# gundoganalperen/DIRAL

Measured on AMD Instinct MI355X. Metric: agent-steps/sec (envs x vehicles), 64-UE/32-res batched env, higher is better.
Workload: dtype f64

## Files before the change

diral_amd/_lib.py:

```python
from __future__ import annotations

import ctypes
import os

from .config import DiralCfg

HERE = os.path.dirname(os.path.abspath(__file__))
LIB_PATH = os.environ.get("DIRAL_LIB") or os.path.join(HERE, "libdiral_env.so")

SYMBOLS = [
    "diral_cfg_defaults", "diral_env_state_space", "diral_env_validate", "diral_env_strerror",
    "diral_env_abi_version", "diral_env_create", "diral_env_destroy", "diral_env_hbm_bytes",
    "diral_env_reset", "diral_env_step", "diral_env_observe", "diral_env_update_velocity",
    "diral_env_sample", "diral_env_info_age", "diral_env_export_state", "diral_env_import_state",
    "diral_env_metrics", "diral_env_check", "diral_env_last_hip_error", "diral_sps_step", "diral_sps_init",
    "diral_env_set_trace", "diral_env_set_option", "diral_env_last_kernel",
    "diral_sps_window_from_chobs", "diral_sps_step_chobs", "diral_driver_shape",
    "diral_env_export_entries", "diral_env_import_entries",
    "diral_env_set_clock", "diral_clock_add", "diral_sps_step_chobs_clocked", "diral_env_step_policy",
    "diral_env_set_capture_rotation", "diral_env_align_phase",
    "diral_env_export_prev_obs", "diral_env_import_prev_obs", "diral_env_prefill", "diral_env_prefill_mode",
    "diral_env_rollout",
]

_lib = None


class DiralLibraryError(RuntimeError):
    pass


def load() -> ctypes.CDLL:
    global _lib
    if _lib is not None:
        return _lib
# ... 32 lines not shown
        "diral_env_last_hip_error": (ctypes.c_char_p, [P]),
        "diral_sps_step": (I, [I, I, P, P, P, D, D, D, P, P, P, U64, P, P]),
        "diral_sps_init": (I, [I, I, P, P, U64, P]),
        "diral_env_set_trace": (I, [P, P, I, I, P]),
        "diral_env_set_option": (I, [P, I, I64]),
        "diral_env_last_kernel": (I, [P]),
        "diral_sps_window_from_chobs": (I, [I, I, P, I, P, P, P]),
        "diral_sps_step_chobs": (I, [I, I, P, I, P, P, P, D, D, D, P, P, P, U64, P, P]),
        "diral_driver_shape": (I, [I, I, I, P, I, P, P, P, P, P, I, I, D, P, P, P, P, P, P]),
        "diral_env_set_clock": (I, [P, P]),
        "diral_clock_add": (I, [P, I64, P]),
        "diral_sps_step_chobs_clocked": (I, [I, I, P, I, P, P, P, D, D, D, U64, P, P, P]),
        "diral_env_step_policy": (I, [P, I, P, I64, P, P, P, P, I, P, P]),
        "diral_env_set_capture_rotation": (I, [P, I, P]),
        "diral_env_align_phase": (I, [P, I, P]),
        "diral_env_export_prev_obs": (I, [P, P, P]),
        "diral_env_import_prev_obs": (I, [P, P, P]),
        "diral_env_prefill": (I, [P, P, I, U64, P, I, P, P, P, D, D, P]),
        "diral_env_prefill_mode": (I, [P, I, P, I, U64, P, I, P, P, P, D, D, P]),
        "diral_env_rollout": (I, [P, I, P, I, I64, P, I, P, P, I, P, P]),
    }
    for name in SYMBOLS:
        try:
            fn = getattr(lib, name)
        except AttributeError as exc:
            raise DiralLibraryError("libdiral_env.so lacks symbol %s" % name) from exc
        fn.restype, fn.argtypes = sig[name]
    from .config import ABI_VERSION
    got = int(lib.diral_env_abi_version())
    if got != ABI_VERSION:
# ... 9 lines not shown
```

diral_amd/csrc/diral_env.hip:

```cpp
#include <hip/hip_runtime.h>

#include <cmath>
#include <cstdio>
#include <cstdlib>
#include <cstring>
#include <string>
#include <vector>

#include "aux_kernels.hpp"
#include "common.hpp"
#include "launch.hpp"
#include "observe_kernel.hpp"
#include "piggyback_kernel.hpp"
#include "posdist_kernel.hpp"
#include "step_params.hpp"

using namespace diral;

struct DevBuf {
  void* p;
  size_t bytes;
  size_t reset_bytes;
  int fill;
};
constexpr int kNoFill = -1;
constexpr bool kOnReset = true;

struct Hooks {
  int table_form = 0;
  bool no_fast64 = false;
  bool no_wide = false;
  bool slow_first = true;
  bool wide_slow_first = false;
  int f32_margin = -1;
};

struct DiralEnv {
  DiralCfg cfg;
  Hooks hooks;
  std::vector<DevBuf> bufs;
  int B = 0, N = 0, A = 0, K = 0, S = 0, NV = 0, NR = 0, vpl = 1;
  int device = 0;
  StepParams base;
  RichParams rich;
  uint32_t lds_bytes = 0;
  int64_t env_offset = 0;
  int kernel_path = DIRAL_PATH_AUTO;
  int last_kernel = -1;
  double* pos_x = nullptr;
  double* pos_y = nullptr;
  double* vel = nullptr;
  uint32_t* tkey = nullptr;
  double* tx = nullptr;
  double* ring = nullptr;
  bool plane_valid = true, ring_valid = false;
  uint32_t* tcode = nullptr;
  uint32_t* tage = nullptr;
  uint32_t* tseq = nullptr;
  uint32_t* told = nullptr;
  uint32_t* slow = nullptr;
  uint64_t slow_launches = 0;
  bool capture_rotates = false;
  int32_t* la = nullptr;
  int32_t* pf = nullptr;
  double* metrics = nullptr;
  uint32_t* err = nullptr;
  double* edges = nullptr;
  double* edges1 = nullptr;
  double* inv_tab = nullptr;
  double* trace = nullptr;
  int trace_len = 0, trace_per_env = 0;
  bool flat_y = true;
  uint32_t* yflag = nullptr;
  int off_chobs_pb = -1;
  double* prev_obs = nullptr;
  double* obs_new = nullptr;
  int32_t* txid = nullptr;
// ... 72 lines not shown
  const int vpl = vpl_for(c->num_users);
  return lds_layout(64 * vpl, c->num_channels, c->num_bins > 0 ? c->num_bins : 1, vpl, 4 * vpl).total > 160u * 1024u;
}
bool runs_large(const DiralEnv* e) { return e->large || e->kernel_path == DIRAL_PATH_LARGE; }

bool fits_fast64(const DiralEnv* e) { return !e->large && e->vpl == 1 && e->NV == 64 && e->A <= kFastMaxA; }
bool fits_wide(const DiralEnv* e) { return !e->large && e->vpl > 1 && e->A <= kWideMaxA; }

Hooks read_hooks() {
  Hooks h;
  if (const char* f = std::getenv("DIRAL_TABLE_FORM")) h.table_form = std::strcmp(f, "packed") == 0 ? 1 : (std::strcmp(f, "plane") == 0 ? -1 : 0);
  h.no_fast64 = std::getenv("DIRAL_NO_FAST64") != nullptr;
  h.no_wide = std::getenv("DIRAL_NO_WIDE") != nullptr;
  if (const char* off = std::getenv("DIRAL_NO_SLOW_FIRST")) h.slow_first = off[0] != '1';
  if (const char* ws = std::getenv("DIRAL_WIDE_SLOW_FIRST")) h.wide_slow_first = ws[0] == '1';
  if (const char* fm = std::getenv("DIRAL_F32_MARGIN")) h.f32_margin = std::max(0, std::atoi(fm));
  return h;
}

constexpr double kPackedMinNeighbours = 20.0;
constexpr double kPackedMinNeighbours2 = 15.0;
bool use_packed_table(const DiralEnv* e) {
  if (e->vpl == 1) return true;
  if (e->hooks.table_form != 0) return e->hooks.table_form > 0;
  const double neigh = e->N * 2.0 * e->cfg.communication_range / e->cfg.highway_length;
  return neigh >= (e->vpl == 2 ? kPackedMinNeighbours2 : kPackedMinNeighbours);
}

int device_of_ptr(const void* p) {
  hipPointerAttribute_t a;
// ... 238 lines not shown
  f.chobs_mode = (p.chobs_out ? 1 : 0) | ((p.mode == DIRAL_STEP_MY_STEP && p.state_type == 2) ? 2 : 0);
  f.L = p.L; f.Rc = p.Rc; f.Rb = p.Rb; f.inv_w = p.hist_inv_width; f.t = p.t; f.t_dev = p.t_dev;
  f.actions = p.actions; f.pos_x = p.pos_x; f.pos_y = p.pos_y; f.vel = p.vel; f.tkey = p.tkey; f.tx = p.tx;
  f.metrics = p.metrics; f.err = p.err; f.edges = p.edges; f.inv_tab = e->inv_tab;
  f.ring = d.use_ring ? e->ring : nullptr;
  f.tcode = e->tcode; f.tage = e->tage; f.tseq = e->tseq; f.told = e->told;
  f.la = d.la;
  f.trace_len = p.trace_len; f.trace_per_env = p.trace_per_env;
  f.state_out = p.state_out; f.rew_out = p.rew_out;
  f.done_out = p.done_out; f.dbg = p.dbg;
  f.B = p.B;
  f.f32_m16 = d.use_fast64 ? f32_margin16(p.L, p.Rb, p.K, e->hooks.f32_margin) : 0;
  f.f32_xmax = (float)p.L;
  f.slow_cnt_r = nullptr; f.slow_list_r = nullptr; f.slow_flag_r = nullptr;
  f.slow_cnt_w = nullptr; f.slow_list_w = nullptr; f.slow_flag_w = nullptr; f.slow_cnt_z = nullptr;
  return f;
}

void rotate_slow_sets(DiralEnv* e, FastParams& f, hipStream_t s) {
  const size_t w = slow_set_words(e);
  uint32_t* const set_r = e->slow + (e->slow_launches % 3) * w;
  uint32_t* const set_w = e->slow + ((e->slow_launches + 1) % 3) * w;
  uint32_t* const set_z = e->slow + ((e->slow_launches + 2) % 3) * w;
  f.slow_cnt_r = set_r; f.slow_list_r = set_r + 16; f.slow_flag_r = set_r + 16 + fast_slow_max(e->B);
  if (e->capture_rotates || !stream_is_capturing(s)) {
    f.slow_cnt_w = set_w; f.slow_list_w = set_w + 16; f.slow_flag_w = set_w + 16 + fast_slow_max(e->B);
    f.slow_cnt_z = set_z;
    ++e->slow_launches;
  }
}

hipError_t launch_step_any(DiralEnv* e, const StepParams& p, const StepPlan& d, hipStream_t s, const PolParams* pol = nullptr) {
  const hipError_t st = d.use_ring ? ensure_ring(e, s) : ensure_plane(e, s);
  if (st != hipSuccess) return st;
  if (d.use_ring) e->plane_valid = false;
  else if (p.mode != kModeObserve) e->ring_valid = false;
  e->last_kernel = d.last_kernel;
  if (d.launch == StepLaunch::Large) return launch_large(p, e->lg, s);
  if (d.launch == StepLaunch::General) return launch_general(e->vpl, d.general_fast, p, e->lds_bytes, s);
  FastParams f = fast_params(e, p, d);
  if (d.slow_sets) rotate_slow_sets(e, f, s);
  RichParams r = rich_for(e, p);
  r.chobs_out = p.chobs_out;
  r.pf = ((p.flags & DIRAL_F_PROPORTIONAL_FAIR) && p.mode == DIRAL_STEP_MY_STEP) ? p.pf : nullptr;
  r.pf_threshold = p.pf_threshold; r.pf_penalty = p.pf_penalty;
  const int grid = p.B + (d.slow_sets ? fast_slow_max(p.B) : 0);
  switch (d.launch) {
    case StepLaunch::WideSlots: return launch_wide_slots(f, r, *pol, d.k, e->vpl, p.B, s);
    case StepLaunch::Wide: return e->vpl == 2 ? launch_wide2(f, r, d.k, grid, s) : launch_wide4(f, r, d.k, grid, s);
    case StepLaunch::Fast64Slots: return launch_fast64_slots(f, r, *pol, d.k.ch, d.k.out64, p.B, s);
    case StepLaunch::Fast64Policy: return launch_fast64_policy(f, r, *pol, d.k.out64, grid, s);
    default: return launch_fast64(f, r, d.k, grid, s);
  }
}

hipError_t launch_posdist_if_needed(DiralEnv* e, const StepParams& p, hipStream_t s) {
  const bool full = (p.flags & DIRAL_F_ADD_POSDIST) != 0;
  const bool type1 = (p.flags & DIRAL_F_ADD_POSDIST_PIGGY) && p.posdist_type == 1;
  if (!p.state_out || !(full || type1)) return hipSuccess;
  PosdistParams q;
  q.N = p.N; q.A = p.A; q.K = p.K; q.S = p.S; q.NV = p.NV; q.NR = p.NR; q.flags = p.flags;
// ... 196 lines not shown
  CREATE_TRY(own(e, e->pos_y, bn * 8));
  CREATE_TRY(own(e, e->vel, bn * 8));
  const size_t tab_slack = 512 + 64 * 256;
  CREATE_TRY(own(e, e->tkey, tab * 4, tab_slack * 4, kOnReset));
  CREATE_TRY(own(e, e->tx, tab * 8, tab_slack * 8, kOnReset));
  if (fits_fast64(e) || fits_wide(e)) {
    CREATE_TRY(own(e, e->ring, (size_t)e->B * e->NR * 8 * 8, 0, kOnReset));
    if (use_packed_table(e)) {
      const size_t nq = (size_t)e->B * (e->NR / 4);
      CREATE_TRY(own(e, e->tcode, nq * e->NV * 4, 512 * 4, kOnReset));
      CREATE_TRY(own(e, e->tage, nq * e->NV * 4, 512 * 4, kOnReset));
      CREATE_TRY(own(e, e->tseq, (size_t)e->B * e->NR * 4, 64 * 4, kOnReset));
      CREATE_TRY(own(e, e->told, nq * 4, 16 * 4, kOnReset));
    }
    CREATE_TRY(own(e, e->slow, 3 * slow_set_words(e) * 4, 0, kOnReset));
    e->ring_valid = true;
  }
  CREATE_TRY(own(e, e->metrics, (size_t)e->B * DIRAL_M_COLUMNS * 8, 0, kOnReset));
  CREATE_TRY(own(e, e->err, 4));
  CREATE_TRY(own(e, e->yflag, 4, 0, false, kNoFill));
  CREATE_TRY(own(e, e->edges, (size_t)(e->K + 1) * 8, 0, false, kNoFill));
  CREATE_TRY(own(e, e->edges1, (size_t)(e->K + 1) * 8, 0, false, kNoFill));
  CREATE_TRY(own(e, e->inv_tab, 256 * 8, 0, false, kNoFill));
  if (has(cfg, DIRAL_F_TRACK_ARRIVAL)) CREATE_TRY(own(e, e->la, bn * e->N * 4, 0, kOnReset, 0xFF));
  if (has(cfg, DIRAL_F_PROPORTIONAL_FAIR)) CREATE_TRY(own(e, e->pf, bn * 4, 0, kOnReset));
  if (has(cfg, DIRAL_F_PIGGYBACKING)) {
    if (piggy_search_lds_bytes(e->N) > 48u * 1024u)
      CREATE_TRY(hipFuncSetAttribute(reinterpret_cast<const void*>(piggy_search_kernel), hipFuncAttributeMaxDynamicSharedMemorySize,
                                     (int)piggy_search_lds_bytes(e->N)));
    CREATE_TRY(own(e, e->prev_obs, bn * e->A * 8, 0, kOnReset));
// ... 66 lines not shown
  r.off_act = off.act; r.off_chobs = has(cfg, DIRAL_F_PIGGYBACKING) ? -1 : off.chobs; r.off_hist = off.hist; r.off_rew = off.rew; r.off_idx = off.idx;
  r.off_skip = 0; r.len_skip = 0;
  r.off_pos = off.pos; r.off_vel = off.vel; r.off_fp = off.fp;
  r.H = cfg->highway_height; r.vel = e->vel; r.pos_y = e->pos_y;
  if (e->hooks.no_fast64 && e->vpl == 1) e->kernel_path = DIRAL_PATH_GENERAL;
  if (e->hooks.no_wide && e->vpl > 1 && !e->large) e->kernel_path = DIRAL_PATH_GENERAL;
  *out = e;
  return DIRAL_OK;
}

int diral_env_destroy(DiralEnv* e) {
  if (!e) return DIRAL_OK;
  DeviceGuard guard(e->device);
  for (const DevBuf& b : e->bufs) (void)hipFree(b.p);
  if (e->trace) (void)hipFree(e->trace);
  if (e->dbg) (void)hipFree(e->dbg);
  delete e;
  return DIRAL_OK;
}

int64_t diral_env_hbm_bytes(const DiralEnv* e) {
  int64_t sum = 0;
  if (e) for (const DevBuf& b : e->bufs) sum += (int64_t)b.bytes;
  return sum;
}

int diral_env_set_option(DiralEnv* e, int option, int64_t value) {
  if (!e) return DIRAL_ERR_BAD_ARG;
  switch (option) {
    case DIRAL_OPT_ENV_OFFSET:
// ... 16 lines not shown
}

int diral_env_last_kernel(const DiralEnv* e) { return e ? e->last_kernel : DIRAL_ERR_BAD_ARG; }

const char* diral_env_last_hip_error(const DiralEnv* e) { return e ? e->last_hip_error.c_str() : ""; }

int diral_env_reset(DiralEnv* e, const double* x0, const double* y0, const double* v0, uint64_t seed,
                    void* stream) {
  if (!e) return DIRAL_ERR_BAD_ARG;
  DEVICE_ENTER(e->device);
  hipStream_t s = (hipStream_t)stream;
  const size_t bn = (size_t)e->B * e->N;
  for (const DevBuf& b : e->bufs)
    if (b.reset_bytes) HIP_TRY(e, hipMemsetAsync(b.p, b.fill, b.reset_bytes, s));
  e->slow_launches = 0;
  e->plane_valid = true; e->ring_valid = e->ring != nullptr;
  HIP_TRY(e, launch_1d<reset_kernel>(bn, s, (int)bn, e->cfg.highway_length, has(&e->cfg, DIRAL_F_MOBILITY_VARY) ? 1 : 0, seed,
                                     (uint64_t)e->env_offset * (uint64_t)e->N, x0, y0, v0, e->pos_x, e->pos_y, e->vel));
  if (y0) { if (refresh_flat_y(e, s) != DIRAL_OK) return DIRAL_ERR_HIP; }
  else e->flat_y = true;
  return DIRAL_OK;
}

int diral_env_step(DiralEnv* e, int mode, const int32_t* actions, int64_t t, void* state_out, void* rew_out,
                   uint8_t* done_out, void* chobs_out, int out_dtype, double episode, double epsilon,
                   void* stream) {
  if (!e || !actions) return DIRAL_ERR_BAD_ARG;
  if (mode != DIRAL_STEP_MY_STEP && mode != DIRAL_STEP_MY_STEP_CH && mode != DIRAL_STEP_DESIGN)
    return DIRAL_ERR_BAD_ARG;
  if (out_dtype != DIRAL_F32 && out_dtype != DIRAL_F64) return DIRAL_ERR_BAD_ARG;
// ... 193 lines not shown
                           const int32_t* tab_seq, const int32_t* tab_age, const double* tab_x,
                           const int32_t* last_arrival, void* stream) {
  if (!e) return DIRAL_ERR_BAD_ARG;
  DEVICE_ENTER(e->device);
  hipStream_t s = (hipStream_t)stream;
  const size_t bn = (size_t)e->B * e->N;
  if (pos_x) HIP_TRY(e, hipMemcpyAsync(e->pos_x, pos_x, bn * 8, hipMemcpyDeviceToDevice, s));
  if (pos_y) {
    HIP_TRY(e, hipMemcpyAsync(e->pos_y, pos_y, bn * 8, hipMemcpyDeviceToDevice, s));
    if (refresh_flat_y(e, s) != DIRAL_OK) return DIRAL_ERR_HIP;
  }
  if (vel) HIP_TRY(e, hipMemcpyAsync(e->vel, vel, bn * 8, hipMemcpyDeviceToDevice, s));
  if (tab_seq || tab_age || tab_x) {
    HIP_TRY(e, ensure_plane(e, s));
    e->ring_valid = false;
    HIP_TRY(e, launch_1d<import_tables_kernel>(bn * e->N, s, e->B, e->N, e->NV, e->NR, tab_seq, tab_age, tab_x, e->tkey, e->tx));
    if (e->ring) { HIP_TRY(e, ensure_ring(e, s)); HIP_TRY(e, verify_ring(e, s)); }
  }
  if (last_arrival) {
    if (!e->la) return DIRAL_ERR_BAD_CONFIG;
    HIP_TRY(e, hipMemcpyAsync(e->la, last_arrival, bn * e->N * 4, hipMemcpyDeviceToDevice, s));
  }
  return DIRAL_OK;
}

int diral_env_export_prev_obs(DiralEnv* e, double* prev_obs, void* stream) {
  if (!e || !prev_obs) return DIRAL_ERR_BAD_ARG;
  if (!e->prev_obs) return DIRAL_ERR_BAD_CONFIG;
  DEVICE_ENTER(e->device);
  HIP_TRY(e, hipMemcpyAsync(prev_obs, e->prev_obs, (size_t)e->B * e->N * e->A * 8, hipMemcpyDeviceToDevice, (hipStream_t)stream));
// ... 11 lines not shown
int diral_env_export_entries(DiralEnv* e, DiralNeighborEntry* entries, void* stream) {
  if (!e || !entries) return DIRAL_ERR_BAD_ARG;
  DEVICE_ENTER(e->device);
  hipStream_t s = (hipStream_t)stream;
  HIP_TRY(e, ensure_plane(e, s));
  HIP_TRY(e, launch_1d<export_entries_kernel>((size_t)e->B * e->N * e->N, s, e->B, e->N, e->NV, e->NR, e->tkey, e->tx, e->pos_y, entries));
  return DIRAL_OK;
}

int diral_env_import_entries(DiralEnv* e, const DiralNeighborEntry* entries, void* stream) {
  if (!e || !entries) return DIRAL_ERR_BAD_ARG;
  DEVICE_ENTER(e->device);
  hipStream_t s = (hipStream_t)stream;
  e->plane_valid = true;
  e->ring_valid = false;
  HIP_TRY(e, launch_1d<import_entries_kernel>((size_t)e->B * e->N * e->N, s, e->B, e->N, e->NV, e->NR, entries, e->tkey, e->tx));
  if (e->ring) { HIP_TRY(e, ensure_ring(e, s)); HIP_TRY(e, verify_ring(e, s)); }
  return DIRAL_OK;
}

int diral_env_set_trace(DiralEnv* e, const double* x_positions, int T, int per_env, void* stream) {
  if (!e || T < 0) return DIRAL_ERR_BAD_ARG;
  DEVICE_ENTER(e->device);
  hipStream_t s = (hipStream_t)stream;
  HIP_TRY(e, hipStreamSynchronize(s));
  if (e->trace) { (void)hipFree(e->trace); e->trace = nullptr; }
  e->trace_len = 0; e->trace_per_env = 0;
  e->base.trace = nullptr; e->base.trace_len = 0; e->base.trace_per_env = 0;
  if (x_positions && T > 0) {
    const size_t n = (size_t)(per_env ? e->B : 1) * T * e->N;
// ... 132 lines not shown
  if (phase) *phase = (int)(e->slow_launches % 3);
  return DIRAL_OK;
}

int diral_env_align_phase(DiralEnv* e, int phase, void* stream) {
  if (!e || phase < 0 || phase > 2) return DIRAL_ERR_BAD_ARG;
  if (!e->slow || (int)(e->slow_launches % 3) == phase) return DIRAL_OK;
  DEVICE_ENTER(e->device);
  hipStream_t s = (hipStream_t)stream;
  if (stream_is_capturing(s)) { e->capture_violation = true; return DIRAL_ERR_CAPTURE; }
  if (hipMemsetAsync(e->slow, 0, buf_of(e, e->slow).bytes, s) != hipSuccess) return DIRAL_ERR_HIP;
  while ((int)(e->slow_launches % 3) != phase) ++e->slow_launches;
  return DIRAL_OK;
}

int diral_sps_init(int agents, int selection_window, int32_t* prev_action, int32_t* counter, uint64_t seed,
                   void* stream) {
  if (agents < 1 || selection_window < 0 || !prev_action || !counter) return DIRAL_ERR_BAD_ARG;
  DEVICE_ENTER(prev_action);
  return hip_status(launch_1d<sps_init_kernel>((size_t)agents, (hipStream_t)stream, agents, selection_window, seed, prev_action, counter));
}

int diral_env_check(DiralEnv* e, void* stream) {
  if (!e) return DIRAL_ERR_BAD_ARG;
  DEVICE_ENTER(e->device);
  uint32_t flags = 0;
  HIP_TRY(e, hipMemcpyAsync(&flags, e->err, 4, hipMemcpyDeviceToHost, (hipStream_t)stream));
  HIP_TRY(e, hipStreamSynchronize((hipStream_t)stream));
  if (flags) HIP_TRY(e, hipMemsetAsync(e->err, 0, 4, (hipStream_t)stream));
  if (flags & kErrAction) return DIRAL_ERR_ACTION_RANGE;
// ... 8 lines not shown
```

diral_amd/csrc/step_fast64_body.inc:

```
template <bool FLAT, bool OUT64, bool CH, bool EXTRA, bool RICH, bool POL = false>
#ifndef DIRAL_FAST_KSLOTS
__global__ __launch_bounds__(256, DIRAL_FAST_MINWAVES) void DIRAL_FAST_KERNEL(const FastParams p, const RichParams r,
                                                                                const PolParams q) {
#else
__global__ __launch_bounds__(256, DIRAL_FAST_MINWAVES_KS) void DIRAL_FAST_KERNEL(const FastParams p, const RichParams r,
                                                                                const PolParams q) {
#endif
#ifndef DIRAL_FAST_KSLOTS
  static_assert(!POL || (RICH && !CH), "the policy epilogue needs the staged channel observation of a my_step slot");
#else
  static_assert(!POL || (RICH && FLAT && !EXTRA), "the policy epilogue needs the staged channel observation of a my_step / my_step_ch slot");
#endif
  extern __shared__ __align__(16) unsigned char smem[];
#ifndef DIRAL_FAST_KSLOTS
  const FastLds lay = fast_lds_layout(p.K, p.A, RICH, OUT64, FLAT, CH || EXTRA);
#else
  const FastLds lay = fast_lds_layout(p.K, p.A, RICH, OUT64, FLAT, CH || EXTRA, POL);
#endif
  double* s_rv = reinterpret_cast<double*>(smem + lay.rv);
  double* s_edges = reinterpret_cast<double*>(smem + lay.edges);
  unsigned long long* s_mask = reinterpret_cast<unsigned long long*>(smem + lay.mask);
  int* s_act = reinterpret_cast<int*>(smem + lay.act);
  unsigned int* s_hist = reinterpret_cast<unsigned int*>(smem + lay.hist);
  unsigned int* s_cnt = reinterpret_cast<unsigned int*>(smem + lay.cnt);
// ... 2 lines not shown
  mtab_t* s_mtab = reinterpret_cast<mtab_t*>(smem + lay.mtab);
  out_t* s_stage = reinterpret_cast<out_t*>(smem + lay.stage);
  double* s_rtx = reinterpret_cast<double*>(smem + lay.rtx);
  int* s_inr = reinterpret_cast<int*>(smem + lay.inr);
  double* s_px = reinterpret_cast<double*>(smem + lay.px);
  double* s_py = reinterpret_cast<double*>(smem + lay.py);
  double* s_npx = reinterpret_cast<double*>(smem + lay.npx);
  double* s_rew = reinterpret_cast<double*>(smem + lay.rew);
  const int MS = fast_mtab_stride(p.A);
  const int SA = fast_stage_stride(p.A);

  int b = blockIdx.x;
  unsigned int listed = 0u;
  unsigned int* const s_slow = reinterpret_cast<unsigned int*>(smem + lay.slow);
  if (p.slow_cnt_r) {
    const int smax = fast_slow_max(p.B);
    if (blockIdx.x < (unsigned int)smax) {
      if (blockIdx.x >= *p.slow_cnt_r) return;
      b = (int)p.slow_list_r[blockIdx.x];
    } else {
      b = (int)blockIdx.x - smax;
      listed = p.slow_flag_r[b];
    }
  }
  const int tid = threadIdx.x;
  const int lane = tid & 63;
  const int wave = __builtin_amdgcn_readfirstlane(tid >> 6);
  const int N = p.N, A = p.A, K = p.K;
  const int KP = fast_hist_stride(K);
  const size_t bN = (size_t)b * N;
  const bool live = lane < N;
  constexpr int NV = 64;
  DIRAL_FSTAMP(0);
#ifdef DIRAL_TIMING
  if (tid == 0 && p.dbg && !listed) p.dbg[(size_t)p.B * 40 + (((size_t)(p.t & 1) * gridDim.x + b) * 2)] = __builtin_amdgcn_s_memrealtime();
  if (lane == 0 && p.dbg && !listed) {
    unsigned int hw, xcc;
// ... 818 lines not shown
    }
  }
#ifdef DIRAL_TIMING
  if (lane == 0 && p.dbg) p.dbg[(size_t)p.B * 48 + (size_t)b * 4 + wave] = dbg_path;
#endif
  DIRAL_FSTAMP(5);
  __syncthreads();
  DIRAL_FSTAMP(6);
  if (tid == 0) {
    const LateFastArgs ls = (LateFastArgs)late_kernarg_base();
    uint32_t* const flag_w = ls->slow_flag_w;
    if (flag_w) {
      unsigned int fl = 0u;
      if (s_slow[0]) {
        const unsigned int pos = atomicAdd(ls->slow_cnt_w, 1u);
        if (pos < (unsigned int)fast_slow_max(ls->B)) { ls->slow_list_w[pos] = (unsigned int)b; fl = 1u; }
      }
      flag_w[b] = fl;
      uint32_t* const set_z = ls->slow_cnt_z;
      set_z[16 + fast_slow_max(ls->B) + b] = 0u;
      if (b == 0) *set_z = 0u;
    }
  }

  if constexpr (POL) {
    if (wave == 1) {
      const LatePolArgs lq = (LatePolArgs)(late_kernarg_base() + kPolArgOffset);
      void* const shaped_out = lq->shaped_out;
      if (shaped_out) {
#ifdef DIRAL_FAST_KSLOTS
        const size_t sB = (size_t)ks * (size_t)p.B;
#endif
        const int sflags = lq->shape_flags;
        const out_t a = live ? (out_t)s_rew[lane] : (out_t)0;
        const out_t sr = np_row_sum_wave(a, N, lane);
        if (lane == 0) {
// ... 188 lines not shown
```

diral_amd/csrc/step_params.hpp:

```cpp
#pragma once
#include "common.hpp"
#include "policy_device.hpp"
#include "rich_out.hpp"

namespace diral {

constexpr int kFastMaxA = 64;
constexpr int kWideMaxA = 64;

struct FastParams {
  int N, A, K, NR;
  int NV;
  uint32_t flags;
  int reward_design, age_limit, episode_interval;
  int design;
  int done_now;
  int notab;
  int nomove;
  int prr;
  int chobs_mode;
  double L, Rc, Rb, inv_w;
  long long t;
  const long long* t_dev;
  const int32_t* actions;
// ... 16 lines not shown
  const double* inv_tab;
  void* state_out;
  void* rew_out;
  uint8_t* done_out;
  unsigned long long* dbg;
  int B;
  int f32_m16;
  float f32_xmax;
  const uint32_t* slow_cnt_r;
  const uint32_t* slow_list_r;
  const uint32_t* slow_flag_r;
  uint32_t* slow_cnt_w;
  uint32_t* slow_list_w;
  uint32_t* slow_flag_w;
  uint32_t* slow_cnt_z;
};
#ifndef DIRAL_SLOW_SHIFT
#define DIRAL_SLOW_SHIFT 2
#endif
__host__ __device__ inline int fast_slow_max(int B) { const int m = B >> DIRAL_SLOW_SHIFT; return m < 16 ? 16 : (m > 4096 ? 4096 : m); }

typedef const __attribute__((address_space(4))) FastParams* LateFastArgs;
__device__ inline unsigned long long late_kernarg_base() {
  unsigned long long a = (unsigned long long)__builtin_amdgcn_kernarg_segment_ptr();
  asm volatile("" : "+s"(a));
  return a;
}
constexpr unsigned long long kRichArgOffset = (sizeof(FastParams) + alignof(RichParams) - 1) / alignof(RichParams) * alignof(RichParams);
typedef const __attribute__((address_space(4))) RichParams* LateRichArgs;
constexpr unsigned long long kPolArgOffset = (kRichArgOffset + sizeof(RichParams) + alignof(PolParams) - 1) / alignof(PolParams) * alignof(PolParams);
typedef const __attribute__((address_space(4))) PolParams* LatePolArgs;
// ... 14 lines not shown
```

diral_amd/csrc/step_wide_body.inc:

```
template <int VPL, bool OUT64, bool FULL, bool CH, bool EXTRA, bool RICH, bool PACKED>
#ifndef DIRAL_WIDE_KSLOTS
__global__ __launch_bounds__(64 * wide_waves(VPL), VPL == 2 ? (PACKED ? DIRAL_WIDE_MINWAVES2P : DIRAL_WIDE_MINWAVES2) : (PACKED ? DIRAL_WIDE_MINWAVES4P : DIRAL_WIDE_MINWAVES4)) void DIRAL_WIDE_KERNEL(const FastParams p, const RichParams r) {
#else
__global__ __launch_bounds__(64 * wide_waves(VPL), VPL == 2 ? (PACKED ? DIRAL_WIDE_MINWAVES2P : DIRAL_WIDE_MINWAVES2) : (PACKED ? DIRAL_WIDE_MINWAVES4P : DIRAL_WIDE_MINWAVES4)) void DIRAL_WIDE_KERNEL(const FastParams p, const RichParams r,
                                                                                                                  const PolParams q) {
  static_assert(RICH && !CH && !EXTRA, "the policy epilogue needs a my_step slot without the run-time extras");
#endif
  constexpr int NPAD = 64 * VPL, WAVES = wide_waves(VPL), THREADS = 64 * WAVES;
  constexpr int CPW = NPAD / WAVES;
  constexpr int PC = VPL == 2 ? DIRAL_WIDE_PC2 : DIRAL_WIDE_PC4;
  constexpr int NW = PC / 4;
  constexpr int NK = NW * VPL;
  static_assert(PC % 4 == 0 && CPW % PC == 0 && NPAD * NW * 4 <= wide_scratch(VPL) && wide_scratch(VPL) % 16 == 0, "a pass's rank words fill at most the wave's scratch");
  constexpr uint32_t SCR = wide_scratch(VPL);
  static_assert(WAVES >= VPL && WAVES <= 8, "P2 runs on the first VPL waves; the merge loop has 8 per-wave copies");
  static_assert(8 * PC <= 64, "xpos ring: one lane per (column, lag) of a pass");
  constexpr int FIN_UNROLL = VPL == 2 ? 8 : 2;
  constexpr int MT = wide_mtab_stride(VPL);
  static_assert(VPL == 2 || VPL == 4, "one lane holds 2 or 4 viewers");
  typedef typename std::conditional<VPL == 4, uint32_t, uint16_t>::type mword_t;

  extern __shared__ __align__(16) unsigned char smem[];
  auto late_i32 = [](size_t off) -> int {
    return *(const __attribute__((address_space(4))) int*)(late_kernarg_base() + off);
// ... 16 lines not shown
  unsigned long long* s_mask = reinterpret_cast<unsigned long long*>(smem + lay.mask);
  int* s_act = reinterpret_cast<int*>(smem + lay.act);
  unsigned int* s_cnt = reinterpret_cast<unsigned int*>(smem + lay.cnt);
  unsigned int* s_hist = reinterpret_cast<unsigned int*>(smem + lay.hist);
  mword_t* s_mtab = reinterpret_cast<mword_t*>(smem + lay.mtab);
  auto rtx_of = [&](int u) -> double* {
    return reinterpret_cast<double*>(smem + lay.scratch + SCR * (u >> 6)) + (u & 63);
  };
  auto inr_of = [&](int u) -> int* {
    return reinterpret_cast<int*>(smem + lay.scratch + SCR * (u >> 6) + 512u) + (u & 63);
  };

  int b = blockIdx.x;
  unsigned int listed = 0u;
  if (p.slow_cnt_r) {
    const int smax = fast_slow_max(p.B);
    if (blockIdx.x < (unsigned int)smax) {
      if (blockIdx.x >= *p.slow_cnt_r) return;
      b = (int)p.slow_list_r[blockIdx.x];
    } else {
      b = (int)blockIdx.x - smax;
      listed = p.slow_flag_r[b];
    }
  }
  unsigned int* const s_slow = reinterpret_cast<unsigned int*>(smem + lay.slow);
  const int tid = threadIdx.x;
  const int lane = tid & 63;
  const int wave = __builtin_amdgcn_readfirstlane(tid >> 6);
  const int KP = wide_hist_stride(K);
  const size_t bN = (size_t)b * N;
  const size_t bR = (size_t)b * NRows;
  DIRAL_WSTAMP(0);
#ifdef DIRAL_WIDE_KSLOTS
  const int KS = q.K;
#pragma unroll 1
  for (int ks = 0; ks < KS; ++ks) {
  const bool last = ks == KS - 1;
// ... 752 lines not shown
  }

  const unsigned long long late = late_kernarg_base();
  const LateFastArgs lp = (LateFastArgs)late;
#ifndef DIRAL_WIDE_KSLOTS
  void* const state_out = lp->state_out;
#else
  void* const state_out = last ? lp->state_out : nullptr;
#endif
  if (tid == 0) {
    uint32_t* const flag_w = lp->slow_flag_w;
    if (flag_w) {
      unsigned int fl = 0u;
      if (s_slow[0]) {
        const unsigned int pos = atomicAdd(lp->slow_cnt_w, 1u);
        if (pos < (unsigned int)fast_slow_max(lp->B)) { lp->slow_list_w[pos] = (unsigned int)b; fl = 1u; }
      }
      flag_w[b] = fl;
      uint32_t* const set_z = lp->slow_cnt_z;
      set_z[16 + fast_slow_max(lp->B) + b] = 0u;
      if (b == 0) *set_z = 0u;
    }
    uint8_t* const done_out = lp->done_out;
#ifndef DIRAL_WIDE_KSLOTS
    if (done_out) {
      int dn = lp->done_now;
      const long long* const td = lp->t_dev;
      if (td) dn = ((unsigned int)(lp->t + *td) % (unsigned int)lp->episode_interval) == (unsigned int)lp->episode_interval - 1u;
      done_out[b] = (uint8_t)dn;
    }
#else
    if (done_out && last) {
      const long long* const td = lp->t_dev;
      const int dn = ((unsigned int)(lp->t + ks + (td ? *td : 0ll)) % (unsigned int)lp->episode_interval) == (unsigned int)lp->episode_interval - 1u;
      done_out[b] = (uint8_t)dn;
    }
// ... 222 lines not shown
```

diral_amd/vec_env.py:

```python
from __future__ import annotations

import ctypes
from typing import Any, Dict, Mapping, Optional, Tuple, Union

import numpy as np
import torch

from . import _lib
from .config import (DT_F32, DT_F64, ERR_HIP, M_COLUMNS, OK, OPT_ENV_OFFSET, OPT_KERNEL_PATH, PATH_AUTO,
                     PATH_GENERAL, PATH_LARGE, STEP_DESIGN, STEP_MY_STEP, STEP_MY_STEP_CH, ConfigError, EnvConfig)

ENTRY_DTYPE = np.dtype([("pos_x", "<f4"), ("pos_y", "<f4"), ("seq_num", "<i4"), ("last_update", "<i4")])

_MODES = {"my_step": STEP_MY_STEP, "my_step_ch": STEP_MY_STEP_CH, "my_step_design": STEP_DESIGN,
          STEP_MY_STEP: STEP_MY_STEP, STEP_MY_STEP_CH: STEP_MY_STEP_CH, STEP_DESIGN: STEP_DESIGN}


_PARKED: list = []


def _capturing() -> bool:
    try:
        return bool(torch.cuda.is_available() and torch.cuda.is_current_stream_capturing())
    except Exception:
# ... 153 lines not shown
                    or clock.device != self.device or not clock.is_contiguous()):
                raise ValueError("the slot clock must be a contiguous int64 tensor of one element on %s" % (self.device,))
        self._ok(self.lib.diral_env_set_clock(self._h, ctypes.c_void_p(clock.data_ptr()) if clock is not None else None),
                 "diral_env_set_clock")
        self._clock = clock

    def set_capture_rotation(self, on: bool) -> int:
        phase = ctypes.c_int(0)
        self._ok(self.lib.diral_env_set_capture_rotation(self._h, 1 if on else 0, ctypes.byref(phase)),
                 "diral_env_set_capture_rotation")
        return int(phase.value)

    def align_phase(self, phase: int) -> None:
        self._ok(self.lib.diral_env_align_phase(self._h, int(phase), self._stream()), "diral_env_align_phase")

    def last_kernel(self) -> int:
        return int(self.lib.diral_env_last_kernel(self._h))

    def get_total_users(self) -> int:
        return self.N

    def get_num_ch(self) -> int:
        return self.A

    def get_state_space(self) -> int:
        return self.S

    def get_action_space(self) -> int:
        return self.A

# ... 378 lines not shown
```

include/diral_env.h:

```cpp
#ifndef DIRAL_ENV_H
#define DIRAL_ENV_H

#include <stdint.h>

#ifdef __cplusplus
extern "C" {
#endif

#define DIRAL_ABI_VERSION 8

typedef enum DiralStatus {
  DIRAL_OK = 0,
  DIRAL_ERR_BAD_ARG = -1,
  DIRAL_ERR_BAD_CONFIG = -2,
  DIRAL_ERR_UNSUPPORTED = -3,
  DIRAL_ERR_HIP = -4,
  DIRAL_ERR_NO_DEVICE = -5,
  DIRAL_ERR_ACTION_RANGE = -6,
  DIRAL_ERR_SEQ_OVERFLOW = -7,
  DIRAL_ERR_CAPTURE = -8,
  DIRAL_ERR_TABLE_CONFLICT = -9,
  DIRAL_ERR_PIGGY_NO_TX = -10
} DiralStatus;

// ... 220 lines not shown
  double   pen_value;
  void*    shaped_out;
  void*    sum_r_out;
  void*    collision_out;
  int32_t* pen_counter;
  int32_t* pen_prev_actions;
  uint64_t vel_seed;
} DiralRollout;
int diral_env_rollout(DiralEnv* env, int mode, const int32_t* actions_seq, int32_t slots, int64_t t, void* states_out,
                      int states_all, void* rew_out, uint8_t* done_out, int out_dtype, const DiralRollout* rollout,
                      void* stream);

int diral_env_set_clock(DiralEnv* env, const int64_t* t_dev);
int diral_env_set_capture_rotation(DiralEnv* env, int on, int* phase);
int diral_env_align_phase(DiralEnv* env, int phase, void* stream);
int diral_clock_add(int64_t* clock, int64_t inc, void* stream);
int diral_sps_step_chobs_clocked(int agents, int num_channels, const void* chobs, int chobs_dtype,
                                 const int32_t* actions, int32_t* prev_action, int32_t* counter,
                                 double rssi_threshold, double inc_db, double keep_prob, uint64_t seed,
                                 const int64_t* clock, int32_t* actions_out, void* stream);

int diral_sps_init(int agents, int selection_window, int32_t* prev_action, int32_t* counter, uint64_t seed,
                   void* stream);

const char* diral_env_last_hip_error(const DiralEnv* env);

#ifdef __cplusplus
}
#endif
#endif
// ... 1 lines not shown
```

Before: 5.704 billion.

## Size slow-block grid head adaptively from observed slow-set counts

```diff
diff --git a/diral_amd/_lib.py b/diral_amd/_lib.py
--- a/diral_amd/_lib.py
+++ b/diral_amd/_lib.py
@@ -18,7 +18,7 @@
     "diral_sps_window_from_chobs", "diral_sps_step_chobs", "diral_driver_shape",
     "diral_env_export_entries", "diral_env_import_entries",
     "diral_env_set_clock", "diral_clock_add", "diral_sps_step_chobs_clocked", "diral_env_step_policy",
-    "diral_env_set_capture_rotation", "diral_env_align_phase",
+    "diral_env_set_capture_rotation", "diral_env_align_phase", "diral_env_slow_head",
     "diral_env_export_prev_obs", "diral_env_import_prev_obs", "diral_env_prefill", "diral_env_prefill_mode",
     "diral_env_rollout",
 ]
@@ -81,6 +81,7 @@
         "diral_env_step_policy": (I, [P, I, P, I64, P, P, P, P, I, P, P]),
         "diral_env_set_capture_rotation": (I, [P, I, P]),
         "diral_env_align_phase": (I, [P, I, P]),
+        "diral_env_slow_head": (I, [P, P, P, P]),
         "diral_env_export_prev_obs": (I, [P, P, P]),
         "diral_env_import_prev_obs": (I, [P, P, P]),
         "diral_env_prefill": (I, [P, P, I, U64, P, I, P, P, P, D, D, P]),
diff --git a/diral_amd/csrc/diral_env.hip b/diral_amd/csrc/diral_env.hip
--- a/diral_amd/csrc/diral_env.hip
+++ b/diral_amd/csrc/diral_env.hip
@@ -32,6 +32,8 @@
   bool no_wide = false;
   bool slow_first = true;
   bool wide_slow_first = false;
+  bool slow_cap_fixed = false;
+  int slow_cap_force = 0;
   int f32_margin = -1;
 };
 
@@ -61,6 +63,13 @@
   uint32_t* slow = nullptr;
   uint64_t slow_launches = 0;
   bool capture_rotates = false;
+  int slow_cap[3] = {0, 0, 0};
+  uint32_t* slow_seen_host = nullptr;
+  uint32_t* slow_seen_dev = nullptr;
+  uint32_t slow_gen = 1;
+  int slow_hist[4] = {-1, -1, -1, -1};
+  int slow_hist_at = 0;
+  int slow_head_last = 0, slow_cap_last = 0;
   int32_t* la = nullptr;
   int32_t* pf = nullptr;
   double* metrics = nullptr;
@@ -163,6 +172,8 @@
   h.no_wide = std::getenv("DIRAL_NO_WIDE") != nullptr;
   if (const char* off = std::getenv("DIRAL_NO_SLOW_FIRST")) h.slow_first = off[0] != '1';
   if (const char* ws = std::getenv("DIRAL_WIDE_SLOW_FIRST")) h.wide_slow_first = ws[0] == '1';
+  if (const char* cf = std::getenv("DIRAL_SLOW_CAP_FIXED")) h.slow_cap_fixed = cf[0] == '1';
+  if (const char* cc = std::getenv("DIRAL_SLOW_CAP_FORCE")) h.slow_cap_force = std::max(0, std::atoi(cc));
   if (const char* fm = std::getenv("DIRAL_F32_MARGIN")) h.f32_margin = std::max(0, std::atoi(fm));
   return h;
 }
@@ -431,20 +442,51 @@
   f.f32_xmax = (float)p.L;
   f.slow_cnt_r = nullptr; f.slow_list_r = nullptr; f.slow_flag_r = nullptr;
   f.slow_cnt_w = nullptr; f.slow_list_w = nullptr; f.slow_flag_w = nullptr; f.slow_cnt_z = nullptr;
+  f.slow_head = 0; f.slow_cap_w = 0; f.slow_cnt_host = nullptr; f.slow_tag = 0u;
   return f;
 }
 
-void rotate_slow_sets(DiralEnv* e, FastParams& f, hipStream_t s) {
+constexpr int kSlowCapGrowth = 2, kSlowCapFloor = 32, kSlowCapRound = 64, kSlowCapHistory = 4;
+void reset_slow_plan(DiralEnv* e) {
+  e->slow_gen = e->slow_gen % 255u + 1u;
+  for (int i = 0; i < kSlowCapHistory; ++i) e->slow_hist[i] = -1;
+}
+int plan_slow_cap(DiralEnv* e, bool capturing) {
+  const int full = fast_slow_max(e->B);
+  if (capturing || e->hooks.slow_cap_fixed || !e->slow_seen_host) return full;
+  if (e->hooks.slow_cap_force > 0) return std::min(full, e->hooks.slow_cap_force);
+  const uint32_t seen = *(volatile const uint32_t*)e->slow_seen_host;
+  if ((seen >> 24) == e->slow_gen) {
+    e->slow_hist[e->slow_hist_at] = (int)(seen & kSlowCountMask);
+    e->slow_hist_at = (e->slow_hist_at + 1) % kSlowCapHistory;
+  }
+  int most = -1;
+  for (int i = 0; i < kSlowCapHistory; ++i) most = std::max(most, e->slow_hist[i]);
+  if (most < 0) return full;
+  const long long want = ((long long)kSlowCapGrowth * most + kSlowCapFloor + kSlowCapRound - 1) / kSlowCapRound * kSlowCapRound;
+  return (int)std::min<long long>(full, want);
+}
+
+int rotate_slow_sets(DiralEnv* e, FastParams& f, hipStream_t s) {
   const size_t w = slow_set_words(e);
+  const bool capturing = stream_is_capturing(s);
+  const int full = fast_slow_max(e->B);
+  const int head = (capturing || e->hooks.slow_cap_fixed) ? full : e->slow_cap[e->slow_launches % 3];
+  f.slow_head = head;
   uint32_t* const set_r = e->slow + (e->slow_launches % 3) * w;
   uint32_t* const set_w = e->slow + ((e->slow_launches + 1) % 3) * w;
   uint32_t* const set_z = e->slow + ((e->slow_launches + 2) % 3) * w;
   f.slow_cnt_r = set_r; f.slow_list_r = set_r + 16; f.slow_flag_r = set_r + 16 + fast_slow_max(e->B);
-  if (e->capture_rotates || !stream_is_capturing(s)) {
+  if (e->capture_rotates || !capturing) {
     f.slow_cnt_w = set_w; f.slow_list_w = set_w + 16; f.slow_flag_w = set_w + 16 + fast_slow_max(e->B);
     f.slow_cnt_z = set_z;
+    f.slow_cap_w = plan_slow_cap(e, capturing);
+    e->slow_cap[(e->slow_launches + 1) % 3] = f.slow_cap_w;
+    e->slow_cap_last = f.slow_cap_w;
+    if (!capturing) { f.slow_cnt_host = e->slow_seen_dev; f.slow_tag = e->slow_gen << 24; }
     ++e->slow_launches;
   }
+  return head;
 }
 
 hipError_t launch_step_any(DiralEnv* e, const StepParams& p, const StepPlan& d, hipStream_t s, const PolParams* pol = nullptr) {
@@ -456,12 +498,13 @@
   if (d.launch == StepLaunch::Large) return launch_large(p, e->lg, s);
   if (d.launch == StepLaunch::General) return launch_general(e->vpl, d.general_fast, p, e->lds_bytes, s);
   FastParams f = fast_params(e, p, d);
-  if (d.slow_sets) rotate_slow_sets(e, f, s);
+  const int head = d.slow_sets ? rotate_slow_sets(e, f, s) : 0;
+  e->slow_head_last = head;
   RichParams r = rich_for(e, p);
   r.chobs_out = p.chobs_out;
   r.pf = ((p.flags & DIRAL_F_PROPORTIONAL_FAIR) && p.mode == DIRAL_STEP_MY_STEP) ? p.pf : nullptr;
   r.pf_threshold = p.pf_threshold; r.pf_penalty = p.pf_penalty;
-  const int grid = p.B + (d.slow_sets ? fast_slow_max(p.B) : 0);
+  const int grid = p.B + head;
   switch (d.launch) {
     case StepLaunch::WideSlots: return launch_wide_slots(f, r, *pol, d.k, e->vpl, p.B, s);
     case StepLaunch::Wide: return e->vpl == 2 ? launch_wide2(f, r, d.k, grid, s) : launch_wide4(f, r, d.k, grid, s);
@@ -688,6 +731,10 @@
       CREATE_TRY(own(e, e->told, nq * 4, 16 * 4, kOnReset));
     }
     CREATE_TRY(own(e, e->slow, 3 * slow_set_words(e) * 4, 0, kOnReset));
+    for (int i = 0; i < 3; ++i) e->slow_cap[i] = fast_slow_max(e->B);
+    CREATE_TRY(hipHostMalloc((void**)&e->slow_seen_host, 64, hipHostMallocMapped));
+    *e->slow_seen_host = 0u;
+    CREATE_TRY(hipHostGetDevicePointer((void**)&e->slow_seen_dev, e->slow_seen_host, 0));
     e->ring_valid = true;
   }
   CREATE_TRY(own(e, e->metrics, (size_t)e->B * DIRAL_M_COLUMNS * 8, 0, kOnReset));
@@ -784,6 +831,7 @@
   DeviceGuard guard(e->device);
   for (const DevBuf& b : e->bufs) (void)hipFree(b.p);
   if (e->trace) (void)hipFree(e->trace);
+  if (e->slow_seen_host) (void)hipHostFree(e->slow_seen_host);
   if (e->dbg) (void)hipFree(e->dbg);
   delete e;
   return DIRAL_OK;
@@ -830,6 +878,8 @@
   for (const DevBuf& b : e->bufs)
     if (b.reset_bytes) HIP_TRY(e, hipMemsetAsync(b.p, b.fill, b.reset_bytes, s));
   e->slow_launches = 0;
+  for (int i = 0; i < 3; ++i) e->slow_cap[i] = fast_slow_max(e->B);
+  reset_slow_plan(e);
   e->plane_valid = true; e->ring_valid = e->ring != nullptr;
   HIP_TRY(e, launch_1d<reset_kernel>(bn, s, (int)bn, e->cfg.highway_length, has(&e->cfg, DIRAL_F_MOBILITY_VARY) ? 1 : 0, seed,
                                      (uint64_t)e->env_offset * (uint64_t)e->N, x0, y0, v0, e->pos_x, e->pos_y, e->vel));
@@ -1053,6 +1103,7 @@
   if (tab_seq || tab_age || tab_x) {
     HIP_TRY(e, ensure_plane(e, s));
     e->ring_valid = false;
+    reset_slow_plan(e);
     HIP_TRY(e, launch_1d<import_tables_kernel>(bn * e->N, s, e->B, e->N, e->NV, e->NR, tab_seq, tab_age, tab_x, e->tkey, e->tx));
     if (e->ring) { HIP_TRY(e, ensure_ring(e, s)); HIP_TRY(e, verify_ring(e, s)); }
   }
@@ -1094,6 +1145,7 @@
   hipStream_t s = (hipStream_t)stream;
   e->plane_valid = true;
   e->ring_valid = false;
+  reset_slow_plan(e);
   HIP_TRY(e, launch_1d<import_entries_kernel>((size_t)e->B * e->N * e->N, s, e->B, e->N, e->NV, e->NR, entries, e->tkey, e->tx));
   if (e->ring) { HIP_TRY(e, ensure_ring(e, s)); HIP_TRY(e, verify_ring(e, s)); }
   return DIRAL_OK;
@@ -1256,6 +1308,17 @@
   return DIRAL_OK;
 }
 
+int diral_env_slow_head(const DiralEnv* e, int* head, int* cap, int* count) {
+  if (!e) return DIRAL_ERR_BAD_ARG;
+  if (head) *head = e->slow_head_last;
+  if (cap) *cap = e->slow_cap_last;
+  if (count) {
+    const uint32_t seen = e->slow_seen_host ? *(volatile const uint32_t*)e->slow_seen_host : 0u;
+    *count = (e->slow_seen_host && (seen >> 24) == e->slow_gen) ? (int)(seen & kSlowCountMask) : -1;
+  }
+  return DIRAL_OK;
+}
+
 int diral_sps_init(int agents, int selection_window, int32_t* prev_action, int32_t* counter, uint64_t seed,
                    void* stream) {
   if (agents < 1 || selection_window < 0 || !prev_action || !counter) return DIRAL_ERR_BAD_ARG;
diff --git a/diral_amd/csrc/step_fast64_body.inc b/diral_amd/csrc/step_fast64_body.inc
--- a/diral_amd/csrc/step_fast64_body.inc
+++ b/diral_amd/csrc/step_fast64_body.inc
@@ -40,13 +40,14 @@
   unsigned int listed = 0u;
   unsigned int* const s_slow = reinterpret_cast<unsigned int*>(smem + lay.slow);
   if (p.slow_cnt_r) {
-    const int smax = fast_slow_max(p.B);
+    const int smax = p.slow_head;
     if (blockIdx.x < (unsigned int)smax) {
-      if (blockIdx.x >= *p.slow_cnt_r) return;
+      const unsigned int cnt = p.slow_cnt_r[0], cap = p.slow_cnt_r[1];
+      if (blockIdx.x >= (cnt < cap ? cnt : cap)) return;
       b = (int)p.slow_list_r[blockIdx.x];
     } else {
       b = (int)blockIdx.x - smax;
-      listed = p.slow_flag_r[b];
+      listed = (p.slow_flag_r[b] - 1u) < (unsigned int)smax ? 1u : 0u;
     }
   }
   const int tid = threadIdx.x;
@@ -895,12 +896,20 @@
       unsigned int fl = 0u;
       if (s_slow[0]) {
         const unsigned int pos = atomicAdd(ls->slow_cnt_w, 1u);
-        if (pos < (unsigned int)fast_slow_max(ls->B)) { ls->slow_list_w[pos] = (unsigned int)b; fl = 1u; }
+        if (pos < (unsigned int)ls->slow_cap_w) { ls->slow_list_w[pos] = (unsigned int)b; fl = pos + 1u; }
       }
       flag_w[b] = fl;
       uint32_t* const set_z = ls->slow_cnt_z;
       set_z[16 + fast_slow_max(ls->B) + b] = 0u;
-      if (b == 0) *set_z = 0u;
+      if (b == 0) {
+        *set_z = 0u;
+        ls->slow_cnt_w[1] = (unsigned int)ls->slow_cap_w;
+        uint32_t* const cnt_host = ls->slow_cnt_host;
+        if (cnt_host) {
+          const unsigned int c = ls->slow_cnt_r[0];
+          *cnt_host = ls->slow_tag | (c < kSlowCountMask ? c : kSlowCountMask);
+        }
+      }
     }
   }
 
diff --git a/diral_amd/csrc/step_params.hpp b/diral_amd/csrc/step_params.hpp
--- a/diral_amd/csrc/step_params.hpp
+++ b/diral_amd/csrc/step_params.hpp
@@ -54,7 +54,13 @@
   uint32_t* slow_list_w;
   uint32_t* slow_flag_w;
   uint32_t* slow_cnt_z;
+  int slow_head;
+  int slow_cap_w;
+  uint32_t* slow_cnt_host;
+  uint32_t slow_tag;
+  uint32_t slow_pad[3];
 };
+constexpr uint32_t kSlowCountMask = 0x00ffffffu;
 #ifndef DIRAL_SLOW_SHIFT
 #define DIRAL_SLOW_SHIFT 2
 #endif
diff --git a/diral_amd/csrc/step_wide_body.inc b/diral_amd/csrc/step_wide_body.inc
--- a/diral_amd/csrc/step_wide_body.inc
+++ b/diral_amd/csrc/step_wide_body.inc
@@ -54,13 +54,14 @@
   int b = blockIdx.x;
   unsigned int listed = 0u;
   if (p.slow_cnt_r) {
-    const int smax = fast_slow_max(p.B);
+    const int smax = p.slow_head;
     if (blockIdx.x < (unsigned int)smax) {
-      if (blockIdx.x >= *p.slow_cnt_r) return;
+      const unsigned int cnt = p.slow_cnt_r[0], cap = p.slow_cnt_r[1];
+      if (blockIdx.x >= (cnt < cap ? cnt : cap)) return;
       b = (int)p.slow_list_r[blockIdx.x];
     } else {
       b = (int)blockIdx.x - smax;
-      listed = p.slow_flag_r[b];
+      listed = (p.slow_flag_r[b] - 1u) < (unsigned int)smax ? 1u : 0u;
     }
   }
   unsigned int* const s_slow = reinterpret_cast<unsigned int*>(smem + lay.slow);
@@ -843,12 +844,20 @@
       unsigned int fl = 0u;
       if (s_slow[0]) {
         const unsigned int pos = atomicAdd(lp->slow_cnt_w, 1u);
-        if (pos < (unsigned int)fast_slow_max(lp->B)) { lp->slow_list_w[pos] = (unsigned int)b; fl = 1u; }
+        if (pos < (unsigned int)lp->slow_cap_w) { lp->slow_list_w[pos] = (unsigned int)b; fl = pos + 1u; }
       }
       flag_w[b] = fl;
       uint32_t* const set_z = lp->slow_cnt_z;
       set_z[16 + fast_slow_max(lp->B) + b] = 0u;
-      if (b == 0) *set_z = 0u;
+      if (b == 0) {
+        *set_z = 0u;
+        lp->slow_cnt_w[1] = (unsigned int)lp->slow_cap_w;
+        uint32_t* const cnt_host = lp->slow_cnt_host;
+        if (cnt_host) {
+          const unsigned int c = lp->slow_cnt_r[0];
+          *cnt_host = lp->slow_tag | (c < kSlowCountMask ? c : kSlowCountMask);
+        }
+      }
     }
     uint8_t* const done_out = lp->done_out;
 #ifndef DIRAL_WIDE_KSLOTS
diff --git a/diral_amd/vec_env.py b/diral_amd/vec_env.py
--- a/diral_amd/vec_env.py
+++ b/diral_amd/vec_env.py
@@ -191,6 +191,12 @@
     def align_phase(self, phase: int) -> None:
         self._ok(self.lib.diral_env_align_phase(self._h, int(phase), self._stream()), "diral_env_align_phase")
 
+    def slow_head(self) -> Dict[str, int]:
+        head, cap, count = ctypes.c_int(0), ctypes.c_int(0), ctypes.c_int(-1)
+        self._ok(self.lib.diral_env_slow_head(self._h, ctypes.byref(head), ctypes.byref(cap), ctypes.byref(count)),
+                 "diral_env_slow_head")
+        return {"head": int(head.value), "cap": int(cap.value), "count": int(count.value)}
+
     def last_kernel(self) -> int:
         return int(self.lib.diral_env_last_kernel(self._h))
 
diff --git a/include/diral_env.h b/include/diral_env.h
--- a/include/diral_env.h
+++ b/include/diral_env.h
@@ -258,6 +258,7 @@
 int diral_env_set_clock(DiralEnv* env, const int64_t* t_dev);
 int diral_env_set_capture_rotation(DiralEnv* env, int on, int* phase);
 int diral_env_align_phase(DiralEnv* env, int phase, void* stream);
+int diral_env_slow_head(const DiralEnv* env, int* head, int* cap, int* count);
 int diral_clock_add(int64_t* clock, int64_t inc, void* stream);
 int diral_sps_step_chobs_clocked(int agents, int num_channels, const void* chobs, int chobs_dtype,
                                  const int32_t* actions, int32_t* prev_action, int32_t* counter,
```

Result: no change. 5.684 billion (-0.3%).
